# zyj0021200/simpleImageCaptionZoo

Measured on AMD Instinct MI355X. Metric: captions/sec (SCST step), BUTDDetection COCO14-size vocab, higher is better.
Workload: dtype f32

## Files before the change

simpleimagecaptionzoo_amd/csrc/butd.hip:

```cpp
#include <vector>

#include "butd_impl.h"

namespace icz {

int Butd::init(const icz_butd_dims& d) {
    dims = d;
    ICZ_REQUIRE(d.R > 0 && d.R <= 64, "butd: R=%d must be in 1..64 (36 boxes / 49 grid cells)", d.R);
    ICZ_REQUIRE(d.D % 4 == 0 && d.H % 4 == 0 && d.E % 4 == 0 && d.A % 4 == 0, "butd: D,H,E,A must be multiples of 4");
    ICZ_REQUIRE(d.V > 3 && d.max_rows > 0 && d.max_len > 0, "butd: bad V/max_rows/max_len");
    const size_t rows = d.max_rows, H = d.H, D = d.D, E = d.E, A = d.A, V = d.V, R = d.R;
    ICZ_TRY(alloc((void**)&w_enc, sizeof(float) * A * D));
    ICZ_TRY(alloc((void**)&w_dec, sizeof(float) * A * H));
    ICZ_TRY(alloc((void**)&w_aff, sizeof(float) * A));
    const size_t Vp = pad_vocab(d.V);
    ICZ_TRY(alloc((void**)&w_pred, sizeof(float) * Vp * H));
    ICZ_TRY(alloc((void**)&n_enc, sizeof(float) * A));
    ICZ_TRY(alloc((void**)&n_dec, sizeof(float) * A));
    ICZ_TRY(alloc((void**)&n_aff, sizeof(float) * 4));
    ICZ_TRY(alloc((void**)&n_pred, sizeof(float) * V));
    ICZ_TRY(alloc((void**)&mean, sizeof(float) * rows * D));
    ICZ_TRY(alloc((void**)&premean, sizeof(float) * rows * 4 * H));
    ICZ_TRY(alloc((void**)&enc_ctx, sizeof(float) * rows * R * A));
    for (int i = 0; i < 2; ++i) {
        ICZ_TRY(alloc((void**)&h1[i], sizeof(float) * rows * H));
        ICZ_TRY(alloc((void**)&c1[i], sizeof(float) * rows * H));
        ICZ_TRY(alloc((void**)&h2[i], sizeof(float) * rows * H));
        ICZ_TRY(alloc((void**)&c2[i], sizeof(float) * rows * H));
    }
    ICZ_TRY(alloc((void**)&emb, sizeof(float) * rows * E));
    ICZ_TRY(alloc((void**)&ctx, sizeof(float) * rows * D));
    ICZ_TRY(alloc((void**)&scores, sizeof(float) * rows * R));
    ICZ_TRY(alloc((void**)&alpha, sizeof(float) * rows * R));
    ICZ_TRY(alloc((void**)&h2drop, sizeof(float) * rows * H));
    ICZ_TRY(alloc((void**)&logits, sizeof(float) * rows * Vp));
    ICZ_TRY(alloc((void**)&amax_val, sizeof(float) * rows * ARGMAX_PARTS));
    ICZ_TRY(alloc((void**)&amax_idx, sizeof(int) * rows * ARGMAX_PARTS));
    ICZ_TRY(alloc((void**)&it, sizeof(int64_t) * rows));
    ICZ_TRY(alloc_scalars(mem));
    size_t nmax = 4 * H;
    if (A > nmax) nmax = A;
    if (V > nmax) nmax = V;
    ws_floats = (size_t)TARGET_WGS * 4096 * 2 + rows * nmax;
    {
        const size_t kmax = 2 * H + (E > D ? E : D), r128 = rows < 128 ? rows : 128;
        const size_t need = (kmax / 256 + 1) * r128 * 4 * H;
        if (need > ws_floats) ws_floats = need;
    }
    ICZ_TRY(alloc((void**)&ws, sizeof(float) * ws_floats));
    ICZ_TRY(mem.synced());
    if (const char* e = getenv("ICZ_EARLY_OUT")) early_out = atoi(e) != 0;
    if (const char* e = getenv("ICZ_MERGE_SMALL")) { const int n = atoi(e); if (n >= 0 && n <= 32) merge_small = n; }
    return ICZ_OK;
}

int Butd::refresh(hipStream_t st) {
    ICZ_REQUIRE(bound, "butd: parameters not bound");
    const int A = dims.A, D = dims.D, H = dims.H, V = dims.V;
    WeightNormTable wt = {};
    int nb = 0;
    auto add = [&](const float* v, const float* g, float* w, float* norm, int rows, int cols) {
        wt.j[wt.count++] = {v, g, w, norm, rows, cols, nb};
        nb += cdiv(rows, 4);
    };
    add(P.enc_att_v, P.enc_att_g, w_enc, n_enc, A, D);
    add(P.dec_att_v, P.dec_att_g, w_dec, n_dec, A, H);
    add(P.affine_v, P.affine_g, w_aff, n_aff, 1, A);
    add(P.predict_v, P.predict_g, w_pred, n_pred, V, H);
    hipLaunchKernelGGL(weight_norm_multi_kernel, dim3(nb), dim3(256), 0, st, wt);
    ICZ_CHECK_HIP(hipGetLastError());
    fresh = true;
    wt_fresh = false;
    return ICZ_OK;
}

bool Butd::wt_possible() const {
    GemmArgs g = {};
    g.nseg = 1;
    g.seg[0] = {w_enc, w_enc, 4 * dims.H, 4 * dims.H, 4 * dims.H, nullptr};
    g.M = 64; g.N = dims.D + dims.H;
    GemmArgs p = g, q = g;
    p.N = q.N = dims.H;
    p.nseg = 2; p.seg[1] = p.seg[0];
    return dims.H % 64 == 0 && dims.D % 64 == 0 && gemm_resident_x3_fits(g) && gemm_resident_x3_pair_fits(p, q);
// ... 228 lines not shown

using namespace icz;

extern "C" {

int icz_butd_create(const icz_butd_dims* dims, icz_butd_t** out) { return abi_create<Butd>("icz_butd_create", dims, out); }

int icz_butd_destroy(icz_butd_t* h) {
    delete reinterpret_cast<Butd*>(h);
    return ICZ_OK;
}

int icz_butd_bind_params(icz_butd_t* h, const icz_butd_params* p) {
    ICZ_REQUIRE(h && p, "icz_butd_bind_params: null argument");
    ICZ_TRY(check_param_table("icz_butd_bind_params", p, sizeof(*p), (1u << 16) | (1u << 17)));
    Butd* b = reinterpret_cast<Butd*>(h);
    if (b->bound && memcmp(&b->P, p, sizeof(*p)) != 0) {
        ICZ_CHECK_HIP(hipDeviceSynchronize());
        b->gc.clear();
    }
    b->P = *p;
    b->bound = true;
    b->fresh = false;
    return ICZ_OK;
}

int icz_butd_set_option(icz_butd_t* h, const char* name, int32_t value) {
    ICZ_REQUIRE(h && name, "icz_butd_set_option: null argument");
    Butd* b = reinterpret_cast<Butd*>(h);
    if (strcmp(name, "graphs") == 0) { b->use_graphs = value != 0; return ICZ_OK; }
    if (strcmp(name, "concurrent") == 0) { b->concurrent = value != 0; return ICZ_OK; }
    if (strcmp(name, "early_out") == 0) { b->early_out = value != 0; return ICZ_OK; }
    if (strcmp(name, "small_nt") == 0) { b->small_nt = value != 0; return ICZ_OK; }
    if (strcmp(name, "group_att") == 0) { b->group_att = value != 0; return ICZ_OK; }
    if (strcmp(name, "merge_small") == 0) {
        ICZ_REQUIRE(value >= 0 && value <= 32, "icz_butd_set_option: merge_small %d outside 0..32", value);
        b->merge_small = value;
        return ICZ_OK;
    }
    set_error("icz_butd_set_option: unknown option '%s'", name);
    return ICZ_ERR_INVALID;
}

int icz_butd_set_mask_sum_global(icz_butd_t* h, const float* mask_sum_global_dev, void* stream) {
    return set_norm_global("icz_butd_set_mask_sum_global", reinterpret_cast<Butd*>(h), mask_sum_global_dev, stream);
}

int icz_butd_set_grad_callback(icz_butd_t* h, icz_grad_ready_cb cb, void* user) {
    ICZ_REQUIRE(h, "null handle");
    Butd* b = reinterpret_cast<Butd*>(h);
    b->grad_cb = cb; b->grad_cb_user = user;
    return ICZ_OK;
}

int icz_butd_refresh_weights(icz_butd_t* h, void* stream) {
    ICZ_REQUIRE(h, "null handle");
    return reinterpret_cast<Butd*>(h)->refresh((hipStream_t)stream);
}

int icz_butd_greedy(icz_butd_t* h, const float* feats, int32_t B, int32_t max_len, int64_t* ids_out,
                    float* alphas_out, void* stream) {
    ICZ_REQUIRE(h, "null handle");
    return reinterpret_cast<Butd*>(h)->greedy(feats, B, max_len, ids_out, alphas_out, (hipStream_t)stream);
}

int icz_butd_step(icz_butd_t* h, const float* feats, int32_t B, const int64_t* it, float* h1, float* c1,
// ... 22 lines not shown
```

simpleimagecaptionzoo_amd/csrc/butd_impl.h:

```cpp
#pragma once
#include <vector>
#include <stdint.h>

#include "decoder_core.h"

namespace icz {

struct StepIO {
    int rows;
    const float* feats;
    const int32_t* img_of_row;
    int rows_per_img;
    const int64_t* it;
    bool emb_ready;
    const float *h1_in, *c1_in, *h2_in, *c2_in;
    float *h1_out, *c1_out, *h2_out, *c2_out;
    float* emb_out;
    float* gates_td_out;
    float* gates_lm_out;
    float* dec_ctx_out;
    float* alpha_out;
    float* alpha_out2; int alpha2_stride;
    float* ctx_out;
    float* h2drop_out;
    float* logits_out;
    int logits_ld;
    int* pred_nsplit;
    float* ws_alt;
    float* scores_alt;
    DropCfg drop_emb, drop_att, drop_out;
    bool skip_predict;
    const int* live;
};

struct TrainBuf {
    int B = 0, T = 0;
    int64_t* tok = nullptr;
    float *emb = nullptr, *h1 = nullptr, *c1 = nullptr, *h2 = nullptr, *c2 = nullptr;
    float *gtd = nullptr, *glm = nullptr, *dec = nullptr, *alpha = nullptr, *ctx = nullptr, *h2d = nullptr, *logit = nullptr;
    int* nany = nullptr;
    int32_t* img2 = nullptr;
    int32_t* imgk = nullptr;
    float* dEncImg = nullptr;
    float *dGtd = nullptr, *dGlm = nullptr, *dDec = nullptr, *dEmb = nullptr, *dH2d = nullptr, *dEnc = nullptr;
    float *dwaff = nullptr, *dalpha = nullptr, *dS = nullptr, *dGsum = nullptr;
    float *dc1[2] = {nullptr, nullptr}, *dc2[2] = {nullptr, nullptr};
    float* X[4] = {nullptr, nullptr, nullptr, nullptr}; size_t xfloats = 0;
    float *dWp = nullptr, *dWenc = nullptr, *dWdec = nullptr, *dWaff = nullptr, *scalars = nullptr;
    float* wslab[2] = {nullptr, nullptr}; size_t wslab_floats[2] = {0, 0};
};

struct Butd : CaptionHead, DecodeMember {
    static constexpr int TARGET_WGS = 512;
    static constexpr int ATT_PARTS = 4;
    static constexpr int STEP_WGS = 256;
    icz_butd_dims dims;
    icz_butd_params P;
    bool bound = false, fresh = false;
    DeviceBuffers mem;

    float *w_enc = nullptr, *w_dec = nullptr, *w_aff = nullptr, *w_pred = nullptr;
    float *n_enc = nullptr, *n_dec = nullptr, *n_aff = nullptr, *n_pred = nullptr;
    float *mean = nullptr, *premean = nullptr, *enc_ctx = nullptr;
    float *h1[2], *c1[2], *h2[2], *c2[2];
    float *emb = nullptr, *ctx = nullptr, *scores = nullptr, *alpha = nullptr, *h2drop = nullptr, *logits = nullptr;
    int64_t* it = nullptr;
    float* amax_val = nullptr; int* amax_idx = nullptr;
    float* ws = nullptr;
    size_t ws_floats = 0;
    float *wt_lm_ih = nullptr, *wt_lm_hh = nullptr, *wt_td_ih_h2 = nullptr, *wt_td_hh = nullptr;
    bool wt_fresh = false;
    bool wt_possible() const;
    int refresh_transposes(hipStream_t st);

    int alloc(void** p, size_t bytes) { return mem.alloc(p, bytes); }
    int init(const icz_butd_dims& d);
    int refresh(hipStream_t st);
    int gemm_nt(GemmArgs& g, int* nsplit_out, hipStream_t st);
    int prologue(const float* feats, int n_img, hipStream_t st);
    int step(const StepIO& s, hipStream_t st);
    int zero_state(int rows, int which, hipStream_t st);
    int greedy(const float* feats, int B, int max_len, int64_t* ids_out, float* alphas_out, hipStream_t st);

    GraphCache gc{24};
    bool use_graphs = false;
    bool concurrent = true;
    uintptr_t opt_bits() const {
        return (concurrent ? 1 : 0) + (early_out ? 2 : 0) + 4 * merge_small + (small_nt ? 256 : 0) + (group_att ? 512 : 0);
    }
    int greedy_impl(const float* feats, int B, int max_len, int64_t* ids_out, float* alphas_out, hipStream_t st);
    int sample_impl(const float* feats, int B, int T, int64_t* seq_out, float* logp_out, hipStream_t st);
    int greedy_chain(const float* feats, int B, int max_len, int64_t* ids_out, float* alphas_out, hipStream_t st, bool scst = false);
    int sample_chain(const float* feats, int B, int T, int64_t* seq_out, float* logp_out, hipStream_t st, int row0 = 0, int64_t* ids_out = nullptr);
    int rollouts(const float* feats, int B, int T, const icz_rng* r, int64_t* ids_out, int64_t* seq_out, float* logp_out, hipStream_t st);
    int rollouts_impl(const float* feats, int B, int T, int64_t* ids_out, int64_t* seq_out, float* logp_out, hipStream_t st);
    SideStream side;
    SideStream low;
    icz_grad_ready_cb grad_cb = nullptr; void* grad_cb_user = nullptr;
    int sample_backward_impl(const float* reward, const icz_butd_params& G, float* loss_out, float* mask_sum_out, hipStream_t st,
                             int phases = 0xF, bool fire_cb = true);
    bool bptt_joined = false;
    int merge_small = 8;
    int cur_rows = 0, cur_row0 = 0;
    bool early_out = true;
    bool bptt_early_out = false;
    bool small_nt = true;
    int cur_K = 1, cur_nimg = 0;
    bool group_att = false;

    const float* seam_feats = nullptr;
    int vocab() const override { return dims.V; }
    int row_capacity() const override { return dims.max_rows; }
    bool refreshed() const override { return fresh; }
    bool compact_step() const override { return true; }
    EmbSlot emb_slot() const override { return {P.embed_weight, emb, dims.E, 1}; }
    DeviceBuffers& buffers() override { return mem; }
    int prologue(const float* feats, int n_img, int k, const int32_t* img_of_row, hipStream_t st) override;
    int step(int rows, const int64_t* it, const int32_t* img_of_row, int rows_per_img, int cur, bool slabs, LogitsView* out,
             hipStream_t st) override;
    void gather(const int32_t* src_row, int rows, int fan, hipStream_t st) override;

    TrainBuf tb;
    icz_rng rng = {};
    const float* cur_feats = nullptr;
    int ensure_train(int B, int T);
    int train_step(const float* feats, int rows, int Bs, int t, bool train, hipStream_t st, bool emb_ready = false, int* pred_nsplit = nullptr,
                   bool skip_predict = false, const int* live = nullptr, int row0 = 0);
    int sample(const float* feats, int B, int T, const icz_rng* r, int64_t* seq_out, float* logp_out, hipStream_t st);
    int sample_n(const float* feats, int B, int K, int T, const icz_rng* r, int64_t* seq_out, float* logp_out, hipStream_t st);
    int sample_n_impl(const float* feats, int B, int K, int T, int64_t* seq_out, float* logp_out, hipStream_t st);
    int sample_mask_sum(float* out, hipStream_t st);
    int sample_backward(const float* reward, const icz_butd_params* G, float* loss_out, float* mask_sum_out,
                        float mask_sum_global, hipStream_t st);
    int xe_forward(const float* feats, const int64_t* captions, int B, int L, const int32_t* lengths, const icz_rng* r,
                   int train, float* packed_out, hipStream_t st);
    int sample_backward_dlogp(const float* dlogp, const icz_butd_params* G, hipStream_t st);
    int xe_backward_dlogits(const float* dpacked, const icz_butd_params* G, hipStream_t st);
    int xe_backward(float smoothing, const icz_butd_params* G, float* loss_out, float n_tokens_global, hipStream_t st);
    int gemm_auto(GemmLayout layout, GemmArgs& g, float* slab, size_t slab_floats, int* ns_out, hipStream_t st);
// ... 8 lines not shown
```

simpleimagecaptionzoo_amd/csrc/butd_kernels.h:

```cpp
#pragma once
#include <stdlib.h>

#include "icz_common.h"
#include "rng.h"

namespace icz {
namespace {

__global__ __launch_bounds__(256) void weight_norm_kernel(const float* __restrict__ v, const float* __restrict__ g,
                                                          float* __restrict__ w, float* __restrict__ norm,
                                                          int rows, int cols) {
    const int lane = threadIdx.x & 63;
    const int row = blockIdx.x * 4 + (threadIdx.x >> 6);
    if (row >= rows) return;
    const float* vr = v + (size_t)row * cols;
    float ss = 0.f;
    for (int c = lane * 4; c < cols; c += 256) {
        f32x4 x = *reinterpret_cast<const f32x4*>(vr + c);
        ss += x[0] * x[0] + x[1] * x[1] + x[2] * x[2] + x[3] * x[3];
    }
    ss = wave_sum(ss);
    const float nrm = sqrtf(ss);
    const float s = g[row] / nrm;
    float* wr = w + (size_t)row * cols;
// ... 1177 lines not shown
        l[v] = g;
    }
    ls = block_sum_256(ls, smf);
    if (tid == 0) loss_rows[row] = ls;
}

__global__ __launch_bounds__(256) void sum_scale_kernel(const float* __restrict__ x, int n, float scale_host, const float* __restrict__ n_dev,
                                                        float* __restrict__ out) {
    __shared__ float smf[4];
    const float scale = (n_dev && n_dev[0] > 0.f) ? 1.0f / n_dev[0] : scale_host;
    float s = 0.f;
    for (int i = threadIdx.x; i < n; i += 256) s += x[i];
    s = block_sum_256(s, smf);
    if (threadIdx.x == 0) out[0] = s * scale;
}

struct LstmBwdArgs {
    const float* dh_a; int ns_a;
    int lda_a;
    const float* dh_b; int ns_b; int lda_b;
    const float* dh_c; int ns_c; int lda_c;
    const float* dhdrop;
    const float* dc_in;
    const float* gates;
    const float* c_prev;
    const float* c_cur;
    float* dgates;
    float* dc_prev;
    int rows, H;
    int rows_a, rows_b, rows_c;
    int dc_in_rows;
    const int* live;
    const int* carry_live;
};
__global__ __launch_bounds__(256) void lstm_bwd_point_kernel(LstmBwdArgs a, DropCfg dc) {
    const int row = blockIdx.y;
    const int j = blockIdx.x * 256 + threadIdx.x;
    if (j >= a.H) return;
    const int H = a.H, G = 4 * H;
    const int lflag = live_flag(a.live), cflag = live_flag(a.carry_live);
    const float* g = a.gates + (size_t)row * G + j;
    const float gi = g[0], gf = g[H], gg = g[2 * H], go = g[3 * H];
    const float cc = a.c_cur[(size_t)row * H + j];
    const float cp = a.c_prev ? a.c_prev[(size_t)row * H + j] : 0.f;
    float dhd = 0.f;
    if (a.dhdrop) dhd = a.dhdrop[(size_t)row * H + j];
    if (flag_dead(lflag)) {
        float* o = a.dgates + (size_t)row * G + j;
        o[0] = 0.f; o[H] = 0.f; o[2 * H] = 0.f; o[3 * H] = 0.f;
        return;
    }
    const bool carry = cflag != 0;
    float dh = 0.f;
    if (a.dh_a && carry && row < a.rows_a) dh += sum_slabs1(a.dh_a, a.ns_a, (size_t)a.rows_a * a.lda_a, (size_t)row * a.lda_a + j);
    if (a.dh_b && row < a.rows_b) dh += sum_slabs1(a.dh_b, a.ns_b, (size_t)a.rows_b * a.lda_b, (size_t)row * a.lda_b + j);
    if (a.dh_c && row < a.rows_c) dh += sum_slabs1(a.dh_c, a.ns_c, (size_t)a.rows_c * a.lda_c, (size_t)row * a.lda_c + j);
    if (a.dhdrop) {
        float d = dhd;
        if (dc.mode) d = dc.keep((uint64_t)row * H + j) ? d * 2.0f : 0.f;
        dh += d;
    }
    const float dcin = (a.dc_in && carry && row < a.dc_in_rows) ? a.dc_in[(size_t)row * H + j] : 0.f;
    const float tc = tanhf(cc);
    const float dcv = dcin + dh * go * (1.f - tc * tc);
    float* o = a.dgates + (size_t)row * G + j;
    o[0] = dcv * gg * gi * (1.f - gi);
    o[H] = dcv * cp * gf * (1.f - gf);
    o[2 * H] = dcv * gi * (1.f - gg * gg);
    o[3 * H] = dh * tc * go * (1.f - go);
    a.dc_prev[(size_t)row * H + j] = dcv * gf;
}


constexpr int DALPHA_COLS = 512;
__global__ __launch_bounds__(256) void att_bwd_dalpha_kernel(const float* __restrict__ dctx, int ns, int ldc, int rows,
                                                             const float* __restrict__ feats, int R, int D,
                                                             float* __restrict__ dalpha_part, const int* __restrict__ live,
                                                             const int32_t* __restrict__ img_of_row) {
    __shared__ __attribute__((aligned(16))) float sd[DALPHA_COLS];
    const int lflag = live_flag(live);
    const int row = blockIdx.x, part = blockIdx.y, nparts = gridDim.y;
    const int tid = threadIdx.x, lane = tid & 63, wave = tid >> 6;
    const int c0 = part * DALPHA_COLS;
    const size_t ss = (size_t)rows * ldc;
    constexpr int NR = 5;
    const int ca = c0 + 4 * lane, cb = ca + 256;
    const bool va = ca < D, vb = cb < D;
    const float* frow = feats + (size_t)(img_of_row ? img_of_row[row] : row) * R * D;
// ... 634 lines not shown
```

simpleimagecaptionzoo_amd/csrc/butd_train.hip:

```cpp
#include <math.h>

#include "butd_impl.h"

namespace icz {

static inline int round4(int x) { return pad_vocab(x); }

__global__ void sample_init_kernel(uint8_t* unf, int* nunf, int64_t* tok, int B, int T) {
    const int i = blockIdx.x * blockDim.x + threadIdx.x;
    if (i < B) { unf[i] = 1; tok[i] = 1; }
    if (i < T) nunf[i] = 0;
}

int Butd::ensure_train(int B, int T) {
    if (tb.B >= B && tb.T >= T) return ICZ_OK;
    ICZ_REQUIRE(B <= 2 * dims.max_rows, "butd: batch %d exceeds capacity %d", B, dims.max_rows);
    ICZ_REQUIRE(T <= XE_MAX_T, "butd: %d steps exceed the limit of %d", T, XE_MAX_T);
    if (tb.B > B) B = tb.B;
    if (tb.T > T) T = tb.T;
    if (dims.max_len > T) T = dims.max_len;
    if (!mem.training.empty()) {
        ICZ_TRY(mem.release_training(&gc));
        tb = TrainBuf();
        drop_loss_buffers();
// ... 18 lines not shown
    ICZ_TRY(alloc((void**)&tb.c2, sizeof(float) * (TB + B) * H));
    ICZ_TRY(alloc((void**)&tb.gtd, sizeof(float) * TB * 4 * H));
    ICZ_TRY(alloc((void**)&tb.glm, sizeof(float) * TB * 4 * H));
    ICZ_TRY(alloc((void**)&tb.dec, sizeof(float) * TB * A));
    ICZ_TRY(alloc((void**)&tb.alpha, sizeof(float) * TB * R));
    ICZ_TRY(alloc((void**)&tb.ctx, sizeof(float) * TB * D));
    ICZ_TRY(alloc((void**)&tb.h2d, sizeof(float) * TB * H));
    ICZ_TRY(alloc((void**)&tb.logit, sizeof(float) * TB * Vp));
    ICZ_TRY(alloc_loss_buffers(mem, TB, B, T));
    ICZ_TRY(alloc((void**)&tb.nany, sizeof(int) * T));
    ICZ_TRY(alloc((void**)&tb.img2, sizeof(int32_t) * B));
    ICZ_TRY(alloc((void**)&tb.imgk, sizeof(int32_t) * B));
    ICZ_TRY(alloc((void**)&tb.dGtd, sizeof(float) * TB * 4 * H));
    ICZ_TRY(alloc((void**)&tb.dGlm, sizeof(float) * TB * 4 * H));
    ICZ_TRY(alloc((void**)&tb.dDec, sizeof(float) * TB * A));
    ICZ_TRY(alloc((void**)&tb.dEmb, sizeof(float) * TB * E));
    ICZ_TRY(alloc((void**)&tb.dH2d, sizeof(float) * TB * H));
    ICZ_TRY(alloc((void**)&tb.dEnc, sizeof(float) * (size_t)B * R * A));
    ICZ_TRY(alloc((void**)&tb.dEncImg, sizeof(float) * (size_t)(B / 2) * R * A));
    ICZ_TRY(alloc((void**)&tb.dwaff, sizeof(float) * (size_t)B * ATT_PARTS * A));
    ICZ_TRY(alloc((void**)&tb.dalpha, sizeof(float) * (size_t)B * R * cdiv((int)D, DALPHA_COLS)));
    ICZ_TRY(alloc((void**)&tb.dS, sizeof(float) * TB * R));
    ICZ_TRY(alloc((void**)&tb.dGsum, sizeof(float) * (size_t)(B + B / 2) * 4 * H));
    for (int i = 0; i < 2; ++i) {
        ICZ_TRY(alloc((void**)&tb.dc1[i], sizeof(float) * (size_t)B * H));
        ICZ_TRY(alloc((void**)&tb.dc2[i], sizeof(float) * (size_t)B * H));
    }
    tb.xfloats = (size_t)TARGET_WGS * 4096 * 2 + (size_t)B * (D + H);
    {
        const size_t kmax = 2 * H + (E > D ? E : D), r128 = B < 128 ? B : 128;
        const size_t need = (kmax / 256 + 1) * r128 * 4 * H;
        if (need > tb.xfloats) tb.xfloats = need;
    }
    for (int i = 0; i < 4; ++i) ICZ_TRY(alloc((void**)&tb.X[i], sizeof(float) * tb.xfloats));
    ICZ_TRY(alloc((void**)&tb.dWp, sizeof(float) * Vp * H));
    ICZ_TRY(alloc((void**)&tb.dWenc, sizeof(float) * A * D));
    ICZ_TRY(alloc((void**)&tb.dWdec, sizeof(float) * A * H));
    {
        auto slabs = [](size_t M, size_t N, size_t K) { return (size_t)gemm_tn_split_pick((int)M, (int)N, (int)K) * M * N; };
        const size_t side[3] = {slabs(A, H, TB), slabs(A, D, B * R), slabs(Vp, H, TB)}, own = slabs(4 * H, H, TB);
        const size_t direct[3] = {A * H, A * D, Vp * H};
        for (int i = 0; i < 3; ++i)
            if (side[i] > direct[i] && side[i] > tb.wslab_floats[1]) tb.wslab_floats[1] = side[i];
        tb.wslab_floats[0] = tb.wslab_floats[1];
        if (own > 4 * H * H && own > tb.wslab_floats[0]) tb.wslab_floats[0] = own;
        for (int i = 0; i < 2; ++i)
            if (tb.wslab_floats[i]) ICZ_TRY(alloc((void**)&tb.wslab[i], sizeof(float) * tb.wslab_floats[i]));
    }
    ICZ_TRY(alloc((void**)&tb.dWaff, sizeof(float) * A));
    ICZ_TRY(alloc((void**)&tb.scalars, sizeof(float) * 16));
    (void)V;
    ICZ_TRY(mem.synced());
    tb.B = B;
    tb.T = T;
    return ICZ_OK;
}

static DropCfg make_drop(const uint64_t* seed_p, bool train, const uint8_t* base, size_t per_step, uint32_t stream, int t, int row0 = 0) {
    DropCfg d = {0, nullptr, seed_p, stream, (uint32_t)t, row0};
    if (!train) return d;
    if (base) { d.mode = 1; d.mask = base + per_step * t; }
    else d.mode = 2;
    return d;
}

int Butd::train_step(const float* feats, int rows, int Bs, int t, bool train, hipStream_t st, bool emb_ready, int* pred_nsplit, bool skip_predict,
                     const int* live, int row0) {
// ... 301 lines not shown
        ICZ_REQUIRE(slab && gemm_slab_floats(g.M, g.N, g.nsplit) <= slab_floats, "butd: slab buffer too small (%d x %d x %d)", g.nsplit, g.M, g.N);
        g.out = slab; g.ldo = g.N; g.bias = nullptr; g.accumulate = 0;
    }
    if (ns_out) *ns_out = g.nsplit;
    return gemm_f32(layout, g, st);
}

int Butd::wgrad(const float* dY, int ldy, int M, const float* X, int ldx, int N, int K, float* out, int ldo, hipStream_t st, const int* rows_live) {
    float* const slab = tb.wslab[st == low.st ? 1 : 0];
    const size_t slab_floats = tb.wslab_floats[st == low.st ? 1 : 0];
    if (slab && ldo == N) {
        const int ns = gemm_tn_split_pick(M, N, K);
        if (ns > 1 && (size_t)ns * M * N <= slab_floats && ((size_t)M * N) % 4 == 0) {
            ICZ_TRY(gemm_tn_split(dY, ldy, M, X, ldx, N, K, ns, slab, rows_live, st));
            const size_t MN = (size_t)M * N;
            hipLaunchKernelGGL(slab_reduce_kernel, dim3(cdiv((int)(MN / 4), 256)), dim3(256), 0, st, (const float*)slab, ns, MN, N, (const float*)nullptr, out);
            ICZ_CHECK_HIP(hipGetLastError());
            return ICZ_OK;
        }
    }
    GemmArgs g = {};
    g.nseg = 1;
    g.rows_live = rows_live;
    g.seg[0] = {dY, X, ldy, ldx, K, nullptr};
    g.M = M; g.N = N; g.out = out; g.ldo = ldo; g.nsplit = 1;
    return gemm_f32(GEMM_TN, g, st);
}

int Butd::colsum(const float* X, int K, int N, int ldx, float* out, hipStream_t st) {
    hipLaunchKernelGGL(colsum_kernel, dim3(cdiv(N, 32)), dim3(256), 0, st, X, K, N, ldx, out);
    return ICZ_OK;
}

int Butd::bptt_prelude(hipStream_t st) {
    if (wt_lm_ih && !wt_fresh) ICZ_TRY(refresh_transposes(st));
    return ICZ_OK;
}

int Butd::bptt(const icz_butd_params& G, hipStream_t st, int phases, bool fire_cb) {
    const int B = cur_B, T = cur_T, Bs = cur_rows, roff = cur_row0;
    const int H = dims.H, D = dims.D, E = dims.E, A = dims.A, R = dims.R, V = dims.V;
    const int Vp = round4(V);
    const int TB = T * Bs;
    const float* feats = cur_feats;
    const size_t sH = (size_t)Bs * H;
    const int* const rl = (bptt_early_out && early_out) ? live_rows : nullptr;
    const int K = cur_K, n_img = K > 1 ? cur_nimg : B;
    const int32_t* const imgk = K > 1 ? tb.imgk : nullptr;

    ICZ_TRY(low.ensure(true));
    hipEvent_t ev_fork = low.fork[0], ev_join = low.join[0];
    if (phases & 1) {
    bptt_joined = false;
    auto side_branch = [&]() -> int {
        ICZ_CHECK_HIP(hipStreamWaitEvent(low.st, ev_fork, 0));
        hipStream_t sb = concurrent ? low.st : st;
        int s1 = wgrad(tb.logit, Vp, Vp, tb.h2d, H, H, TB, tb.dWp, H, sb, rl);
        hipLaunchKernelGGL(colsum_kernel, dim3(cdiv(V, 32)), dim3(256), 0, sb, tb.logit, TB, V, (int)Vp, G.predict_b);
        hipLaunchKernelGGL(weight_norm_bwd_kernel, dim3(cdiv(V, 4)), dim3(256), 0, sb, tb.dWp, H, P.predict_v, P.predict_g, n_pred,
                           G.predict_v, G.predict_g, V, H);
        ICZ_CHECK_HIP(hipEventRecord(ev_join, sb));
        if (s1 != ICZ_OK) { (void)hipStreamWaitEvent(st, ev_join, 0); return s1; }
        return ICZ_OK;
    };
    ICZ_CHECK_HIP(hipEventRecord(ev_fork, st));
    {
        GemmArgs g = {};
        g.nseg = 1;
        g.seg[0] = {tb.logit, w_pred, Vp, H, Vp, nullptr};
        g.M = TB; g.N = H; g.out = tb.dH2d; g.ldo = H; g.rows_live = rl;
        int ns;
        const int sg = gemm_auto(GEMM_NN, g, ws, ws_floats, &ns, st);
        if (sg != ICZ_OK) return sg;
        if (ns > 1) {
            size_t MN = (size_t)TB * H;
            hipLaunchKernelGGL(slab_reduce_kernel, dim3(cdiv((int)(MN / 4), 256)), dim3(256), 0, st, ws, ns, MN, H, (const float*)nullptr, tb.dH2d);
        }
    }
    ICZ_TRY(side_branch());
    const bool ragged = rows_t[T - 1] < B || roff > 0;
    if (ragged) {
        ICZ_CHECK_HIP(hipMemsetAsync(tb.dGtd, 0, sizeof(float) * (size_t)TB * 4 * H, st));
        ICZ_CHECK_HIP(hipMemsetAsync(tb.dGlm, 0, sizeof(float) * (size_t)TB * 4 * H, st));
        ICZ_CHECK_HIP(hipMemsetAsync(tb.dDec, 0, sizeof(float) * (size_t)TB * A, st));
        ICZ_CHECK_HIP(hipMemsetAsync(tb.dS, 0, sizeof(float) * (size_t)TB * R, st));
    }

    auto loop = [&]() -> int {
    int cur = 0;
    int ns1 = 1, ns2 = 1, ns3 = 1, ns4 = 1;
    int bnext = 0;
    for (int t = T - 1; t >= 0; --t) {
        const int bt = rows_t[t];
        const size_t slot = (size_t)t * Bs + roff;
        const int* const live = (bptt_early_out && early_out && t > 0) ? nunf + (t - 1) : nullptr;
        const int* const carry_live = (bptt_early_out && early_out && t + 1 < T) ? nunf + t : nullptr;
        DropCfg d_out = make_drop(d_seed, cur_train, rng.out_mask, (size_t)B * H, RNG_OUT, t);
        DropCfg d_att = make_drop(d_seed, cur_train, rng.att_mask, (size_t)B * R * A, RNG_ATT, t);
        DropCfg d_off = {0, nullptr, nullptr, 0, 0};
        {
            LstmBwdArgs a = {};
            a.dh_a = bnext ? tb.X[2] : nullptr; a.ns_a = ns3; a.lda_a = H; a.rows_a = bnext;
            a.dhdrop = tb.dH2d + slot * H;
            a.dc_in = bnext ? tb.dc2[cur] : nullptr; a.dc_in_rows = bnext;
            a.gates = tb.glm + slot * 4 * H;
            a.c_prev = tb.c2 + slot * H; a.c_cur = tb.c2 + slot * H + sH;
            a.dgates = tb.dGlm + slot * 4 * H; a.dc_prev = tb.dc2[cur ^ 1];
            a.rows = bt; a.H = H; a.live = live; a.carry_live = carry_live;
            hipLaunchKernelGGL(lstm_bwd_point_kernel, dim3(cdiv(H, 256), bt), dim3(256), 0, st, a, d_out);
        }
        const bool rdg = wt_lm_ih && wt_fresh && bt > 32 && bt <= 64 && gemm_slab_floats(bt, D + H, 4 * H / 256) <= tb.xfloats &&
                         gemm_slab_floats(bt, H, 2 * (4 * H / 256)) <= tb.xfloats;
        const bool tdg = small_nt && wt_lm_ih && wt_fresh && bt <= 32;
        if (rdg) {
            GemmArgs g = {};
            g.nseg = 1;
            g.seg[0] = {tb.dGlm + slot * 4 * H, wt_lm_ih, 4 * H, 4 * H, 4 * H, nullptr};
            g.M = bt; g.N = D + H; g.out = tb.X[0]; g.ldo = D + H; g.live = live;
            g.nsplit = ns1 = gemm_resident_x3_nsplit(g);
            ICZ_REQUIRE(gemm_slab_floats(bt, D + H, ns1) <= tb.xfloats, "butd: slab buffer too small for the dgrad slabs");
            ICZ_TRY(gemm_f32(GEMM_NT, g, st));
        } else if (tdg) {
            GemmArgs g = {};
            g.nseg = 1;
            g.seg[0] = {tb.dGlm + slot * 4 * H, wt_lm_ih, 4 * H, 4 * H, 4 * H, nullptr};
            g.M = bt; g.N = D + H; g.out = tb.X[0]; g.ldo = D + H; g.live = live;
            ICZ_TRY(gemm_auto(GEMM_NT, g, tb.X[0], tb.xfloats, &ns1, st));
        } else {
            GemmArgs g = {};
            g.nseg = 1;
            g.seg[0] = {tb.dGlm + slot * 4 * H, P.lm_w_ih, 4 * H, D + H, 4 * H, nullptr};
            g.M = bt; g.N = D + H; g.out = tb.X[0]; g.ldo = D + H; g.live = live;
            ICZ_TRY(gemm_auto(GEMM_NN, g, tb.X[0], tb.xfloats, &ns1, st));
        }
        {
            const int dparts = cdiv(D, DALPHA_COLS);
            hipLaunchKernelGGL(att_bwd_dalpha_kernel, dim3(bt, dparts), dim3(256), 0, st, tb.X[0], ns1, D + H, bt, feats, R, D, tb.dalpha, live, imgk);
            AttBwdDdecArgs da = {enc_ctx, tb.dec + slot * A, w_aff, tb.alpha + slot * R, tb.dalpha, tb.dDec + slot * A, tb.dS + slot * R, R, A, dparts, live, imgk};
            hipLaunchKernelGGL(att_bwd_ddec_kernel, dim3(bt, cdiv(A, 256)), dim3(256), 0, st, da, d_att);
            GemmArgs g = {};
            g.nseg = 1;
            g.seg[0] = {tb.dDec + slot * A, w_dec, A, H, A, nullptr};
            g.M = bt; g.N = H; g.out = tb.X[1]; g.ldo = H; g.live = live;
            ICZ_TRY(gemm_auto(GEMM_NN, g, tb.X[1], tb.xfloats, &ns2, st));
        }
        {
            LstmBwdArgs a = {};
            a.dh_a = bnext ? tb.X[3] : nullptr; a.ns_a = ns4; a.lda_a = H; a.rows_a = bnext;
            a.dh_b = tb.X[0] + D; a.ns_b = ns1; a.lda_b = D + H; a.rows_b = bt;
            a.dh_c = tb.X[1]; a.ns_c = ns2; a.lda_c = H; a.rows_c = bt;
            a.dc_in = bnext ? tb.dc1[cur] : nullptr; a.dc_in_rows = bnext;
            a.gates = tb.gtd + slot * 4 * H;
            a.c_prev = tb.c1 + slot * H; a.c_cur = tb.c1 + slot * H + sH;
            a.dgates = tb.dGtd + slot * 4 * H; a.dc_prev = tb.dc1[cur ^ 1];
            a.rows = bt; a.H = H; a.live = live; a.carry_live = carry_live;
            hipLaunchKernelGGL(lstm_bwd_point_kernel, dim3(cdiv(H, 256), bt), dim3(256), 0, st, a, d_off);
        }
        if (t > 0 && rdg) {
            GemmArgs g3 = {}, g4 = {};
            g3.nseg = 2;
            g3.seg[0] = {tb.dGlm + slot * 4 * H, wt_lm_hh, 4 * H, 4 * H, 4 * H, nullptr};
            g3.seg[1] = {tb.dGtd + slot * 4 * H, wt_td_ih_h2, 4 * H, 4 * H, 4 * H, nullptr};
            g3.M = bt; g3.N = H; g3.out = tb.X[2]; g3.ldo = H; g3.live = live;
            g4.nseg = 1; g4.live = live;
            g4.seg[0] = {tb.dGtd + slot * 4 * H, wt_td_hh, 4 * H, 4 * H, 4 * H, nullptr};
            g4.M = bt; g4.N = H; g4.out = tb.X[3]; g4.ldo = H;
            ns3 = gemm_resident_x3_nsplit(g3); ns4 = gemm_resident_x3_nsplit(g4);
            ICZ_REQUIRE(gemm_slab_floats(bt, H, ns3) <= tb.xfloats, "butd: slab buffer too small for the dgrad slabs");
            ICZ_TRY(gemm_resident_x3_pair(g3, g4, st));
        } else if (t > 0 && tdg) {
            {
                GemmArgs g = {};
                g.nseg = 2;
                g.seg[0] = {tb.dGlm + slot * 4 * H, wt_lm_hh, 4 * H, 4 * H, 4 * H, nullptr};
                g.seg[1] = {tb.dGtd + slot * 4 * H, wt_td_ih_h2, 4 * H, 4 * H, 4 * H, nullptr};
                g.M = bt; g.N = H; g.out = tb.X[2]; g.ldo = H; g.live = live;
                ICZ_TRY(gemm_auto(GEMM_NT, g, tb.X[2], tb.xfloats, &ns3, st));
            }
            {
                GemmArgs g = {};
                g.nseg = 1;
                g.seg[0] = {tb.dGtd + slot * 4 * H, wt_td_hh, 4 * H, 4 * H, 4 * H, nullptr};
                g.M = bt; g.N = H; g.out = tb.X[3]; g.ldo = H; g.live = live;
                ICZ_TRY(gemm_auto(GEMM_NT, g, tb.X[3], tb.xfloats, &ns4, st));
            }
        } else if (t > 0) {
            {
                GemmArgs g = {};
                g.nseg = 2;
                g.seg[0] = {tb.dGlm + slot * 4 * H, P.lm_w_hh, 4 * H, H, 4 * H, nullptr};
                g.seg[1] = {tb.dGtd + slot * 4 * H, P.td_w_ih, 4 * H, H + D + E, 4 * H, nullptr};
                g.M = bt; g.N = H; g.out = tb.X[2]; g.ldo = H; g.live = live;
                ICZ_TRY(gemm_auto(GEMM_NN, g, tb.X[2], tb.xfloats, &ns3, st));
            }
            {
                GemmArgs g = {};
                g.nseg = 1;
                g.seg[0] = {tb.dGtd + slot * 4 * H, P.td_w_hh, 4 * H, H, 4 * H, nullptr};
                g.M = bt; g.N = H; g.out = tb.X[3]; g.ldo = H; g.live = live;
                ICZ_TRY(gemm_auto(GEMM_NN, g, tb.X[3], tb.xfloats, &ns4, st));
            }
        }
        bnext = bt;
        cur ^= 1;
    }
    return ICZ_OK;
    };
    const int s_loop = loop();
    if (grad_cb || s_loop != ICZ_OK) {
        ICZ_CHECK_HIP(hipStreamWaitEvent(st, ev_join, 0));
        bptt_joined = true;
    }
    if (s_loop != ICZ_OK) return s_loop;
    }
    if ((phases & 1) && grad_cb && fire_cb) grad_cb(grad_cb_user, 0);
    const int ldtd = H + D + E, ldlm = D + H;
    const bool tail_side = phases == 0xF && !grad_cb && concurrent;
    if (tail_side) ICZ_CHECK_HIP(hipEventRecord(low.fork[1], st));
    bool tail_forked = false;
    hipStream_t const main_st = st;
    auto behind_loop = [&]() -> int {
    if (phases & 2) {
    {
        GemmArgs g = {};
        g.nseg = 1;
        g.seg[0] = {tb.dGtd, P.td_w_ih + H + D, 4 * H, H + D + E, 4 * H, nullptr};
        g.M = TB; g.N = E; g.out = tb.dEmb; g.ldo = E; g.rows_live = rl;
        int ns;
        ICZ_TRY(gemm_auto(GEMM_NN, g, ws, ws_floats, &ns, st));
        if (ns > 1) {
            size_t MN = (size_t)TB * E;
            hipLaunchKernelGGL(slab_reduce_kernel, dim3(cdiv((int)(MN / 4), 256)), dim3(256), 0, st, ws, ns, MN, E, (const float*)nullptr, tb.dEmb);
        }
        ICZ_CHECK_HIP(embed_grad_launch(st, tb.tok, TB, tb.dEmb, 1, (size_t)0, tb.emb, cur_train ? 2.0f : 1.0f, E, G.embed_weight, V, 1, rl));
    }
// ... 200 lines not shown
```

simpleimagecaptionzoo_amd/csrc/gemm_f32.h:

```cpp
#pragma once
#include "icz_common.h"

namespace icz {

constexpr int GEMM_MAX_SEG = 4;
constexpr int GEMM_BM = 64, GEMM_BN = 64, GEMM_BK = 64;

enum GemmLayout { GEMM_NT = 0, GEMM_NN = 1, GEMM_TN = 2 };

struct GemmSeg {
    const float* A;
    const float* B;
    int lda, ldb;
    int K;
    const int64_t* gather;
};

struct GemmArgs {
    GemmSeg seg[GEMM_MAX_SEG];
    int nseg;
    int M, N;
    float* out;
    int ldo;
    const float* bias;
    int nsplit;
    int chunks_per_split;
    int accumulate;
    int spread;
    const int* live;
    const int* rows_live;
};

int gemm_f32(GemmLayout layout, const GemmArgs& a, hipStream_t stream);
int gemm_route(GemmLayout layout, const GemmArgs& a);
int gemm_pick_split(const GemmArgs& a, int target_wgs, GemmLayout layout = GEMM_NT);
int gemm_pick_split_balanced(const GemmArgs& a, GemmLayout layout, size_t slab_capacity_floats);
size_t gemm_slab_floats(int M, int N, int nsplit);
int gemm_normalize_split(GemmLayout layout, const GemmArgs& a, int nsplit);
int gemm_fit_split(GemmLayout layout, const GemmArgs& a, int nsplit, size_t capacity_floats);

bool gemm_resident_x3_fits(const GemmArgs& a);
int gemm_resident_x3_stages(const GemmArgs& a);
int gemm_resident_x3_nsplit(const GemmArgs& a);
int gemm_resident_x3(const GemmArgs& a, hipStream_t stream);
bool gemm_resident_x3_pair_fits(const GemmArgs& a, const GemmArgs& b);
int gemm_resident_x3_pair(const GemmArgs& a, const GemmArgs& b, hipStream_t stream);
int gemm_predict(const float* x, int H, const float* w_pred, const float* bias, int rows, int V, int Vp, float* logits, int ldl,
                 float* ws, size_t ws_cap_floats, int* pred_nsplit, hipStream_t st, const int* live = nullptr);

int gemm_big_x3(GemmLayout layout, const GemmArgs& a, int cfg, hipStream_t stream);
int gemm_big_cfg(GemmLayout layout, const GemmArgs& a);
int gemm_big_switch();
void gemm_set_big_cfg(int cfg);
constexpr int GEMM_MAX_COLGROUPS = 4;
struct GemmColGroup { const float* B; int ldb; int cols; float* out; int ldo; };
bool gemm_tn_grouped_fits(int M, int K, const GemmColGroup* groups, int ngroups);
int gemm_tn_grouped(const float* dY, int ldy, int M, int K, const GemmColGroup* groups, int ngroups, const int* rows_live, hipStream_t stream);

int gemm_tn_split_pick(int M, int N, int K);
int gemm_tn_split(const float* dY, int ldy, int M, const float* X, int ldx, int N, int K, int nsplit, float* slabs, const int* rows_live, hipStream_t st);
struct GemmSwitches { bool tn_x3, nn_x3, nt_x3big, resident_x3, resident_m128, predict_slabs, resident_k512; unsigned prof_every; int big_cfg; };
const GemmSwitches& gemm_switches();

}
```

simpleimagecaptionzoo_amd/csrc/gemm_resident_x3.hip:

```cpp
#include <stdlib.h>

#include <type_traits>

#include "gemm_f32.h"

namespace icz {

template <int I, int N, class F>
__device__ __forceinline__ void sk_static_for(F&& f) {
    if constexpr (I < N) {
        f(std::integral_constant<int, I>{});
        sk_static_for<I + 1, N>(f);
    }
}

typedef __attribute__((ext_vector_type(8))) __bf16 sk_bf16x8;
typedef __attribute__((ext_vector_type(4))) uint32_t sk_u32x4;
typedef __attribute__((ext_vector_type(2))) uint32_t sk_u32x2;

__device__ __forceinline__ uint32_t sk_cvt_pk_bf16(float lo, float hi) {
    uint32_t r;
    asm("v_cvt_pk_bf16_f32 %0, %1, %2" : "=v"(r) : "v"(lo), "v"(hi));
    return r;
}
// ... 551 lines not shown
    if (!attr) {
        ICZ_CHECK_HIP(hipFuncSetAttribute(reinterpret_cast<const void*>(gemm_resident_x3_m128_kernel<3, STAMPS>), hipFuncAttributeMaxDynamicSharedMemorySize, (int)lds));
        attr = true;
    }
    hipLaunchKernelGGL((gemm_resident_x3_m128_kernel<3, STAMPS>), dim3(cdiv(a.N, 256) * a.nsplit), dim3(256), lds, stream, a);
    ICZ_CHECK_HIP(hipGetLastError());
    return ICZ_OK;
}

#ifdef ICZ_DEV
static unsigned long long* g_sk_stamps = nullptr;
static int rs_dev_env(const char* name) { const char* e = getenv(name); return e ? atoi(e) : 0; }
#endif

int gemm_resident_x3(const GemmArgs& a_in, hipStream_t stream) {
    GemmArgs a = a_in;
    const int nsr = gemm_resident_x3_stages(a);
    ICZ_REQUIRE(rs_shape_ok(a) && a.nsplit == gemm_resident_x3_nsplit(a) && a.chunks_per_split == nsr,
                "gemm_resident_x3: launch does not match the kernel's fixed decomposition (nsplit %d)", a.nsplit);
    ICZ_REQUIRE(a.nsplit > 1 || a.ldo >= a.N, "gemm_resident_x3: output row stride %d below N = %d", a.ldo, a.N);
#ifdef ICZ_DEV
    if (rs_dev_env("ICZ_DEV_STAMPS")) {
        if (!g_sk_stamps) ICZ_CHECK_HIP(hipMalloc((void**)&g_sk_stamps, sizeof(unsigned long long) * 32 * 4096));
        a.bias = reinterpret_cast<const float*>(g_sk_stamps);
        return a.M > 64 ? rs_launch_m128<true>(a, stream) : (nsr == 8 ? rs_launch_k512<true>(a, stream) : rs_launch<4, true>(a, stream));
    }
#endif
    return a.M > 64 ? rs_launch_m128<false>(a, stream) : (nsr == 8 ? rs_launch_k512<false>(a, stream) : rs_launch<4, false>(a, stream));
}

bool gemm_resident_x3_pair_fits(const GemmArgs& a, const GemmArgs& b) {
    return a.M <= 64 && b.M <= 64 && rs_shape_ok(a) && rs_shape_ok(b) && gemm_resident_x3_stages(a) == gemm_resident_x3_stages(b) && a.N >= 512 && b.N >= 512;
}
int gemm_resident_x3_pair(const GemmArgs& a_in, const GemmArgs& b_in, hipStream_t stream) {
    ICZ_REQUIRE(gemm_resident_x3_pair_fits(a_in, b_in), "gemm_resident_x3_pair: shapes outside the kernel's decomposition");
    GemmPair g;
    g.a = a_in; g.b = b_in;
    const int nsr = gemm_resident_x3_stages(g.a), tilew = nsr == 8 ? 128 : 256;
    for (GemmArgs* p : {&g.a, &g.b}) {
        p->nsplit = gemm_resident_x3_nsplit(*p);
        p->chunks_per_split = nsr;
        p->bias = nullptr;
        ICZ_REQUIRE(p->out && p->nsplit > 1, "gemm_resident_x3_pair: slab output expected");
    }
    g.first = cdiv(g.a.N, tilew) * g.a.nsplit;
    constexpr size_t lds = rs_lds_bytes<4, 4>();
    static bool attr = false;
    if (!attr) {
        ICZ_CHECK_HIP(hipFuncSetAttribute(reinterpret_cast<const void*>(gemm_resident_x3_pair_kernel<4, 4, 2, 3>), hipFuncAttributeMaxDynamicSharedMemorySize, (int)lds));
        ICZ_CHECK_HIP(hipFuncSetAttribute(reinterpret_cast<const void*>(gemm_resident_x3_pair_kernel<4, 8, 1, RS_K512_D, 4>), hipFuncAttributeMaxDynamicSharedMemorySize, (int)lds));
        attr = true;
    }
    const dim3 grid(g.first + cdiv(g.b.N, tilew) * g.b.nsplit);
    if (nsr == 8) hipLaunchKernelGGL((gemm_resident_x3_pair_kernel<4, 8, 1, RS_K512_D, 4>), grid, dim3(256), lds, stream, g);
    else hipLaunchKernelGGL((gemm_resident_x3_pair_kernel<4, 4, 2, 3>), grid, dim3(256), lds, stream, g);
    ICZ_CHECK_HIP(hipGetLastError());
    return ICZ_OK;
}

int gemm_predict(const float* x, int H, const float* w_pred, const float* bias, int rows, int V, int Vp, float* logits, int ldl,
                 float* ws, size_t ws_cap_floats, int* pred_nsplit, hipStream_t st, const int* live) {
    GemmArgs g = {};
    g.nseg = 1;
    g.live = live;
    g.seg[0] = {x, w_pred, H, H, H, nullptr};
    g.M = rows; g.N = Vp; g.out = ws; g.ldo = Vp;
    if (gemm_switches().predict_slabs && pred_nsplit && ws && gemm_resident_x3_fits(g) && gemm_resident_x3_nsplit(g) > 1 &&
        gemm_slab_floats(rows, Vp, gemm_resident_x3_nsplit(g)) <= ws_cap_floats) {
        g.nsplit = gemm_resident_x3_nsplit(g);
        *pred_nsplit = g.nsplit;
    } else {
        g.N = V; g.out = logits; g.ldo = ldl; g.bias = bias;
        g.nsplit = 1;
        if (pred_nsplit) *pred_nsplit = 1;
    }
    return gemm_f32(GEMM_NT, g, st);
}

}

#ifdef ICZ_DEV
extern "C" int icz_debug_skinny_stamps(unsigned long long* out_host, int n_workgroups) {
    if (!icz::g_sk_stamps || n_workgroups > 4096) return -1;
    return hipMemcpy(out_host, icz::g_sk_stamps, sizeof(unsigned long long) * 32 * n_workgroups, hipMemcpyDeviceToHost) == hipSuccess ? 0 : -2;
}
#endif
```

Baseline: 11870.

## Pair the LM dgrad GEMM with its h2 recurrent GEMM and widen small-grid pairs in BPTT

In the backward-through-time loop, the LM-gate recurrent dgrad (dGlm x W_lm_hh) is now computed together with the input dgrad in one paired resident GEMM launch. Its slabs go to a new fifth buffer and are consumed one step later by the LSTM pointwise kernel through a carry-gated input. The top-down pair GEMMs can also pick a new K256 single-tile form that launches more workgroups when the auto grid would use less than half the step workgroups. The aim is fewer launches and better occupancy for small-batch backward steps, at the cost of an extra slab buffer, a new kernel instantiation, and changes to how the carry logic consumes the slabs.

New measurement: 11950 (median of 6 runs). Within noise of the previous version (+0.7%).

```diff
diff --git a/simpleimagecaptionzoo_amd/csrc/butd.hip b/simpleimagecaptionzoo_amd/csrc/butd.hip
--- a/simpleimagecaptionzoo_amd/csrc/butd.hip
+++ b/simpleimagecaptionzoo_amd/csrc/butd.hip
@@ -50,6 +50,7 @@
     ICZ_TRY(alloc((void**)&ws, sizeof(float) * ws_floats));
     ICZ_TRY(mem.synced());
     if (const char* e = getenv("ICZ_EARLY_OUT")) early_out = atoi(e) != 0;
+    if (const char* e = getenv("ICZ_BPTT_WIDE")) bptt_wide = atoi(e) != 0;
     if (const char* e = getenv("ICZ_MERGE_SMALL")) { const int n = atoi(e); if (n >= 0 && n <= 32) merge_small = n; }
     return ICZ_OK;
 }
@@ -344,6 +345,7 @@
     if (strcmp(name, "concurrent") == 0) { b->concurrent = value != 0; return ICZ_OK; }
     if (strcmp(name, "early_out") == 0) { b->early_out = value != 0; return ICZ_OK; }
     if (strcmp(name, "small_nt") == 0) { b->small_nt = value != 0; return ICZ_OK; }
+    if (strcmp(name, "bptt_wide") == 0) { b->bptt_wide = value != 0; return ICZ_OK; }
     if (strcmp(name, "group_att") == 0) { b->group_att = value != 0; return ICZ_OK; }
     if (strcmp(name, "merge_small") == 0) {
         ICZ_REQUIRE(value >= 0 && value <= 32, "icz_butd_set_option: merge_small %d outside 0..32", value);
diff --git a/simpleimagecaptionzoo_amd/csrc/butd_impl.h b/simpleimagecaptionzoo_amd/csrc/butd_impl.h
--- a/simpleimagecaptionzoo_amd/csrc/butd_impl.h
+++ b/simpleimagecaptionzoo_amd/csrc/butd_impl.h
@@ -45,7 +45,7 @@
     float *dGtd = nullptr, *dGlm = nullptr, *dDec = nullptr, *dEmb = nullptr, *dH2d = nullptr, *dEnc = nullptr;
     float *dwaff = nullptr, *dalpha = nullptr, *dS = nullptr, *dGsum = nullptr;
     float *dc1[2] = {nullptr, nullptr}, *dc2[2] = {nullptr, nullptr};
-    float* X[4] = {nullptr, nullptr, nullptr, nullptr}; size_t xfloats = 0;
+    float* X[5] = {nullptr, nullptr, nullptr, nullptr, nullptr}; size_t xfloats = 0;
     float *dWp = nullptr, *dWenc = nullptr, *dWdec = nullptr, *dWaff = nullptr, *scalars = nullptr;
     float* wslab[2] = {nullptr, nullptr}; size_t wslab_floats[2] = {0, 0};
 };
@@ -86,7 +86,7 @@
     bool use_graphs = false;
     bool concurrent = true;
     uintptr_t opt_bits() const {
-        return (concurrent ? 1 : 0) + (early_out ? 2 : 0) + 4 * merge_small + (small_nt ? 256 : 0) + (group_att ? 512 : 0);
+        return (concurrent ? 1 : 0) + (early_out ? 2 : 0) + 4 * merge_small + (small_nt ? 256 : 0) + (group_att ? 512 : 0) + (bptt_wide ? 1024 : 0);
     }
     int greedy_impl(const float* feats, int B, int max_len, int64_t* ids_out, float* alphas_out, hipStream_t st);
     int sample_impl(const float* feats, int B, int T, int64_t* seq_out, float* logp_out, hipStream_t st);
@@ -105,6 +105,8 @@
     bool early_out = true;
     bool bptt_early_out = false;
     bool small_nt = true;
+    bool bptt_wide = true;
+    int bptt_pair_form(const GemmArgs& a, const GemmArgs& b, int rows) const;
     int cur_K = 1, cur_nimg = 0;
     bool group_att = false;
 
diff --git a/simpleimagecaptionzoo_amd/csrc/butd_kernels.h b/simpleimagecaptionzoo_amd/csrc/butd_kernels.h
--- a/simpleimagecaptionzoo_amd/csrc/butd_kernels.h
+++ b/simpleimagecaptionzoo_amd/csrc/butd_kernels.h
@@ -1233,6 +1233,7 @@
     int dc_in_rows;
     const int* live;
     const int* carry_live;
+    int b_carry;
 };
 __global__ __launch_bounds__(256) void lstm_bwd_point_kernel(LstmBwdArgs a, DropCfg dc) {
     const int row = blockIdx.y;
@@ -1254,7 +1255,7 @@
     const bool carry = cflag != 0;
     float dh = 0.f;
     if (a.dh_a && carry && row < a.rows_a) dh += sum_slabs1(a.dh_a, a.ns_a, (size_t)a.rows_a * a.lda_a, (size_t)row * a.lda_a + j);
-    if (a.dh_b && row < a.rows_b) dh += sum_slabs1(a.dh_b, a.ns_b, (size_t)a.rows_b * a.lda_b, (size_t)row * a.lda_b + j);
+    if (a.dh_b && (carry || !a.b_carry) && row < a.rows_b) dh += sum_slabs1(a.dh_b, a.ns_b, (size_t)a.rows_b * a.lda_b, (size_t)row * a.lda_b + j);
     if (a.dh_c && row < a.rows_c) dh += sum_slabs1(a.dh_c, a.ns_c, (size_t)a.rows_c * a.lda_c, (size_t)row * a.lda_c + j);
     if (a.dhdrop) {
         float d = dhd;
diff --git a/simpleimagecaptionzoo_amd/csrc/butd_train.hip b/simpleimagecaptionzoo_amd/csrc/butd_train.hip
--- a/simpleimagecaptionzoo_amd/csrc/butd_train.hip
+++ b/simpleimagecaptionzoo_amd/csrc/butd_train.hip
@@ -74,7 +74,7 @@
         const size_t need = (kmax / 256 + 1) * r128 * 4 * H;
         if (need > tb.xfloats) tb.xfloats = need;
     }
-    for (int i = 0; i < 4; ++i) ICZ_TRY(alloc((void**)&tb.X[i], sizeof(float) * tb.xfloats));
+    for (int i = 0; i < 5; ++i) ICZ_TRY(alloc((void**)&tb.X[i], sizeof(float) * tb.xfloats));
     ICZ_TRY(alloc((void**)&tb.dWp, sizeof(float) * Vp * H));
     ICZ_TRY(alloc((void**)&tb.dWenc, sizeof(float) * A * D));
     ICZ_TRY(alloc((void**)&tb.dWdec, sizeof(float) * A * H));
@@ -442,6 +442,13 @@
     return ICZ_OK;
 }
 
+int Butd::bptt_pair_form(const GemmArgs& a, const GemmArgs& b, int rows) const {
+    if (gemm_resident_x3_pair_grid(a, b, RS_PAIR_AUTO) > STEP_WGS / 2) return RS_PAIR_AUTO;
+    const int na = gemm_resident_x3_pair_nsplit(a, RS_PAIR_K256_ONE_TILE), nb = gemm_resident_x3_pair_nsplit(b, RS_PAIR_K256_ONE_TILE);
+    if (gemm_slab_floats(rows, a.N, na) > tb.xfloats || gemm_slab_floats(rows, b.N, nb) > tb.xfloats) return RS_PAIR_AUTO;
+    return RS_PAIR_K256_ONE_TILE;
+}
+
 int Butd::bptt_prelude(hipStream_t st) {
     if (wt_lm_ih && !wt_fresh) ICZ_TRY(refresh_transposes(st));
     return ICZ_OK;
@@ -498,8 +505,9 @@
 
     auto loop = [&]() -> int {
     int cur = 0;
-    int ns1 = 1, ns2 = 1, ns3 = 1, ns4 = 1;
+    int ns1 = 1, ns2 = 1, ns3 = 1, ns4 = 1, ns5 = 1;
     int bnext = 0;
+    bool x5_behind = false;
     for (int t = T - 1; t >= 0; --t) {
         const int bt = rows_t[t];
         const size_t slot = (size_t)t * Bs + roff;
@@ -511,6 +519,9 @@
         {
             LstmBwdArgs a = {};
             a.dh_a = bnext ? tb.X[2] : nullptr; a.ns_a = ns3; a.lda_a = H; a.rows_a = bnext;
+            if (bnext && x5_behind) {
+                a.dh_b = tb.X[4]; a.ns_b = ns5; a.lda_b = H; a.rows_b = bnext; a.b_carry = 1;
+            }
             a.dhdrop = tb.dH2d + slot * H;
             a.dc_in = bnext ? tb.dc2[cur] : nullptr; a.dc_in_rows = bnext;
             a.gates = tb.glm + slot * 4 * H;
@@ -522,6 +533,25 @@
         const bool rdg = wt_lm_ih && wt_fresh && bt > 32 && bt <= 64 && gemm_slab_floats(bt, D + H, 4 * H / 256) <= tb.xfloats &&
                          gemm_slab_floats(bt, H, 2 * (4 * H / 256)) <= tb.xfloats;
         const bool tdg = small_nt && wt_lm_ih && wt_fresh && bt <= 32;
+        GemmArgs gA2 = {}, gB1 = {}, gB2 = {};
+        bool wide = false;
+        int formB = RS_PAIR_AUTO;
+        if (rdg && bptt_wide && t > 0) {
+            GemmArgs gA1 = {};
+            gA1.nseg = gA2.nseg = gB1.nseg = gB2.nseg = 1;
+            gA1.seg[0] = {tb.dGlm + slot * 4 * H, wt_lm_ih, 4 * H, 4 * H, 4 * H, nullptr};
+            gA2.seg[0] = {tb.dGlm + slot * 4 * H, wt_lm_hh, 4 * H, 4 * H, 4 * H, nullptr};
+            gB1.seg[0] = {tb.dGtd + slot * 4 * H, wt_td_ih_h2, 4 * H, 4 * H, 4 * H, nullptr};
+            gB2.seg[0] = {tb.dGtd + slot * 4 * H, wt_td_hh, 4 * H, 4 * H, 4 * H, nullptr};
+            gA1.M = gA2.M = gB1.M = gB2.M = bt;
+            gA1.N = D + H; gA2.N = gB1.N = gB2.N = H;
+            gA2.out = tb.X[4]; gB1.out = tb.X[2]; gB2.out = tb.X[3];
+            gA2.ldo = gB1.ldo = gB2.ldo = H;
+            gA2.live = gB1.live = gB2.live = live;
+            wide = gemm_resident_x3_pair_fits(gA1, gA2) && gemm_resident_x3_pair_fits(gB1, gB2) &&
+                   gemm_slab_floats(bt, H, gemm_resident_x3_pair_nsplit(gA2, RS_PAIR_AUTO)) <= tb.xfloats;
+            if (wide) formB = bptt_pair_form(gB1, gB2, bt);
+        }
         if (rdg) {
             GemmArgs g = {};
             g.nseg = 1;
@@ -529,7 +559,12 @@
             g.M = bt; g.N = D + H; g.out = tb.X[0]; g.ldo = D + H; g.live = live;
             g.nsplit = ns1 = gemm_resident_x3_nsplit(g);
             ICZ_REQUIRE(gemm_slab_floats(bt, D + H, ns1) <= tb.xfloats, "butd: slab buffer too small for the dgrad slabs");
-            ICZ_TRY(gemm_f32(GEMM_NT, g, st));
+            if (wide) {
+                ns5 = gemm_resident_x3_pair_nsplit(gA2, RS_PAIR_AUTO);
+                ICZ_REQUIRE(gemm_slab_floats(bt, H, ns5) <= tb.xfloats, "butd: slab buffer too small for the d h2 slabs of the LM gates");
+                ICZ_TRY(gemm_resident_x3_pair(g, gA2, st));
+            } else
+                ICZ_TRY(gemm_f32(GEMM_NT, g, st));
         } else if (tdg) {
             GemmArgs g = {};
             g.nseg = 1;
@@ -566,7 +601,12 @@
             a.rows = bt; a.H = H; a.live = live; a.carry_live = carry_live;
             hipLaunchKernelGGL(lstm_bwd_point_kernel, dim3(cdiv(H, 256), bt), dim3(256), 0, st, a, d_off);
         }
-        if (t > 0 && rdg) {
+        if (wide) {
+            ns3 = gemm_resident_x3_pair_nsplit(gB1, formB); ns4 = gemm_resident_x3_pair_nsplit(gB2, formB);
+            ICZ_REQUIRE(gemm_slab_floats(bt, H, ns3) <= tb.xfloats && gemm_slab_floats(bt, H, ns4) <= tb.xfloats,
+                        "butd: slab buffer too small for the dgrad slabs");
+            ICZ_TRY(gemm_resident_x3_pair(gB1, gB2, st, formB));
+        } else if (t > 0 && rdg) {
             GemmArgs g3 = {}, g4 = {};
             g3.nseg = 2;
             g3.seg[0] = {tb.dGlm + slot * 4 * H, wt_lm_hh, 4 * H, 4 * H, 4 * H, nullptr};
@@ -611,6 +651,7 @@
                 ICZ_TRY(gemm_auto(GEMM_NN, g, tb.X[3], tb.xfloats, &ns4, st));
             }
         }
+        x5_behind = wide;
         bnext = bt;
         cur ^= 1;
     }
diff --git a/simpleimagecaptionzoo_amd/csrc/gemm_f32.h b/simpleimagecaptionzoo_amd/csrc/gemm_f32.h
--- a/simpleimagecaptionzoo_amd/csrc/gemm_f32.h
+++ b/simpleimagecaptionzoo_amd/csrc/gemm_f32.h
@@ -44,7 +44,10 @@
 int gemm_resident_x3_nsplit(const GemmArgs& a);
 int gemm_resident_x3(const GemmArgs& a, hipStream_t stream);
 bool gemm_resident_x3_pair_fits(const GemmArgs& a, const GemmArgs& b);
-int gemm_resident_x3_pair(const GemmArgs& a, const GemmArgs& b, hipStream_t stream);
+enum GemmPairForm { RS_PAIR_AUTO = 0, RS_PAIR_K256_ONE_TILE = 1 };
+int gemm_resident_x3_pair_nsplit(const GemmArgs& a, int form);
+int gemm_resident_x3_pair_grid(const GemmArgs& a, const GemmArgs& b, int form);
+int gemm_resident_x3_pair(const GemmArgs& a, const GemmArgs& b, hipStream_t stream, int form = RS_PAIR_AUTO);
 int gemm_predict(const float* x, int H, const float* w_pred, const float* bias, int rows, int V, int Vp, float* logits, int ldl,
                  float* ws, size_t ws_cap_floats, int* pred_nsplit, hipStream_t st, const int* live = nullptr);
 
diff --git a/simpleimagecaptionzoo_amd/csrc/gemm_resident_x3.hip b/simpleimagecaptionzoo_amd/csrc/gemm_resident_x3.hip
--- a/simpleimagecaptionzoo_amd/csrc/gemm_resident_x3.hip
+++ b/simpleimagecaptionzoo_amd/csrc/gemm_resident_x3.hip
@@ -607,13 +607,27 @@
 bool gemm_resident_x3_pair_fits(const GemmArgs& a, const GemmArgs& b) {
     return a.M <= 64 && b.M <= 64 && rs_shape_ok(a) && rs_shape_ok(b) && gemm_resident_x3_stages(a) == gemm_resident_x3_stages(b) && a.N >= 512 && b.N >= 512;
 }
-int gemm_resident_x3_pair(const GemmArgs& a_in, const GemmArgs& b_in, hipStream_t stream) {
+static int rs_pair_stages(const GemmArgs& a, int form) { return form == RS_PAIR_K256_ONE_TILE ? 4 : gemm_resident_x3_stages(a); }
+static int rs_pair_tilew(int nsr, int form) { return (form == RS_PAIR_K256_ONE_TILE || nsr == 8) ? 128 : 256; }
+int gemm_resident_x3_pair_nsplit(const GemmArgs& a, int form) {
+    const int nsr = rs_pair_stages(a, form);
+    return nsr > 0 ? rs_total_stages(a) / nsr : 0;
+}
+int gemm_resident_x3_pair_grid(const GemmArgs& a, const GemmArgs& b, int form) {
+    const int nsr = rs_pair_stages(a, form);
+    if (nsr <= 0) return 0;
+    const int tilew = rs_pair_tilew(nsr, form);
+    return cdiv(a.N, tilew) * gemm_resident_x3_pair_nsplit(a, form) + cdiv(b.N, tilew) * gemm_resident_x3_pair_nsplit(b, form);
+}
+int gemm_resident_x3_pair(const GemmArgs& a_in, const GemmArgs& b_in, hipStream_t stream, int form) {
+    ICZ_REQUIRE(form == RS_PAIR_AUTO || form == RS_PAIR_K256_ONE_TILE, "gemm_resident_x3_pair: unknown stage form %d", form);
     ICZ_REQUIRE(gemm_resident_x3_pair_fits(a_in, b_in), "gemm_resident_x3_pair: shapes outside the kernel's decomposition");
     GemmPair g;
     g.a = a_in; g.b = b_in;
-    const int nsr = gemm_resident_x3_stages(g.a), tilew = nsr == 8 ? 128 : 256;
+    const int nsr = rs_pair_stages(g.a, form), tilew = rs_pair_tilew(nsr, form);
     for (GemmArgs* p : {&g.a, &g.b}) {
-        p->nsplit = gemm_resident_x3_nsplit(*p);
+        ICZ_REQUIRE(rs_total_stages(*p) % nsr == 0, "gemm_resident_x3_pair: %d stages do not split into ranges of %d", rs_total_stages(*p), nsr);
+        p->nsplit = rs_total_stages(*p) / nsr;
         p->chunks_per_split = nsr;
         p->bias = nullptr;
         ICZ_REQUIRE(p->out && p->nsplit > 1, "gemm_resident_x3_pair: slab output expected");
@@ -624,10 +638,12 @@
     if (!attr) {
         ICZ_CHECK_HIP(hipFuncSetAttribute(reinterpret_cast<const void*>(gemm_resident_x3_pair_kernel<4, 4, 2, 3>), hipFuncAttributeMaxDynamicSharedMemorySize, (int)lds));
         ICZ_CHECK_HIP(hipFuncSetAttribute(reinterpret_cast<const void*>(gemm_resident_x3_pair_kernel<4, 8, 1, RS_K512_D, 4>), hipFuncAttributeMaxDynamicSharedMemorySize, (int)lds));
+        ICZ_CHECK_HIP(hipFuncSetAttribute(reinterpret_cast<const void*>(gemm_resident_x3_pair_kernel<4, 4, 1, 3>), hipFuncAttributeMaxDynamicSharedMemorySize, (int)lds));
         attr = true;
     }
     const dim3 grid(g.first + cdiv(g.b.N, tilew) * g.b.nsplit);
-    if (nsr == 8) hipLaunchKernelGGL((gemm_resident_x3_pair_kernel<4, 8, 1, RS_K512_D, 4>), grid, dim3(256), lds, stream, g);
+    if (form == RS_PAIR_K256_ONE_TILE) hipLaunchKernelGGL((gemm_resident_x3_pair_kernel<4, 4, 1, 3>), grid, dim3(256), lds, stream, g);
+    else if (nsr == 8) hipLaunchKernelGGL((gemm_resident_x3_pair_kernel<4, 8, 1, RS_K512_D, 4>), grid, dim3(256), lds, stream, g);
     else hipLaunchKernelGGL((gemm_resident_x3_pair_kernel<4, 4, 2, 3>), grid, dim3(256), lds, stream, g);
     ICZ_CHECK_HIP(hipGetLastError());
     return ICZ_OK;
```
